# haiciyang/LaDiffCodec

Hardware: AMD Instinct MI355X
Metric: audio-sec decoded / wall-sec, 16kHz 3kbps 50-step DDPM (higher is better)
Workload: dtype bf16; 1 GPU; LaDiffCodec 3 kbps, diff_dims=256, enc_ratios 8 4, 50-step DDPM, batch=32x2.4 s utterances per GPU; global_batch=32, latent_len=1200, denoise_steps=50, rccl_ranks=1, batches_in_flight=1, parallelism=dp1 (utterance-sharded, no data-path collective)

## Files before the change

ladiffcodec_amd/csrc/attention.hip:

```cpp
#include <algorithm>

#include "ldc_kernels.h"
#include "ldc_math.h"

namespace ldc {

__device__ __forceinline__ float abf2f(unsigned short h) { return __uint_as_float(((unsigned)h) << 16); }
__device__ __forceinline__ unsigned short af2bf(float f) { return hw_bf16(f); }
template <typename T>
__device__ __forceinline__ float ld1(const void* p, size_t i);
template <>
__device__ __forceinline__ float ld1<float>(const void* p, size_t i) { return reinterpret_cast<const float*>(p)[i]; }
template <>
__device__ __forceinline__ float ld1<__bf16>(const void* p, size_t i) {
  return abf2f(reinterpret_cast<const unsigned short*>(p)[i]);
}
template <typename T>
__device__ __forceinline__ void st1(void* p, size_t i, float v);
template <>
__device__ __forceinline__ void st1<float>(void* p, size_t i, float v) { reinterpret_cast<float*>(p)[i] = v; }
template <>
__device__ __forceinline__ void st1<__bf16>(void* p, size_t i, float v) {
  reinterpret_cast<unsigned short*>(p)[i] = af2bf(v);
}
// ... 258 lines not shown
    }
    lf32x16 acc;
#pragma unroll
    for (int r = 0; r < 16; ++r) acc[r] = 0.f;
    acc = mfma_bf16(af[0], bq[0], acc);
    acc = mfma_bf16(af[1], bq[1], acc);
    if (n < L) {
      unsigned short* orow = out + ((size_t)b * L + n) * HD + h * D;
#pragma unroll
      for (int rr = 0; rr < 4; ++rr) {
        const unsigned lo = (unsigned)af2bf(acc[4 * rr]) | ((unsigned)af2bf(acc[4 * rr + 1]) << 16);
        const unsigned hi = (unsigned)af2bf(acc[4 * rr + 2]) | ((unsigned)af2bf(acc[4 * rr + 3]) << 16);
        *reinterpret_cast<uint2*>(orow + 8 * rr + 4 * g) = make_uint2(lo, hi);
      }
    }
  }
}


__device__ __forceinline__ float reduce16_over32(const float (&v)[16], int lane) {
  float a8[8], a4[4], a2[2];
  const bool b4 = lane & 16, b3 = lane & 8, b2 = lane & 4, b1 = lane & 2;
#pragma unroll
  for (int k = 0; k < 8; ++k) a8[k] = (b4 ? v[8 + k] : v[k]) + __shfl_xor(b4 ? v[k] : v[8 + k], 16);
#pragma unroll
  for (int k = 0; k < 4; ++k) a4[k] = (b3 ? a8[4 + k] : a8[k]) + __shfl_xor(b3 ? a8[k] : a8[4 + k], 8);
#pragma unroll
  for (int k = 0; k < 2; ++k) a2[k] = (b2 ? a4[2 + k] : a4[k]) + __shfl_xor(b2 ? a4[k] : a4[2 + k], 4);
  float a1 = (b1 ? a2[1] : a2[0]) + __shfl_xor(b1 ? a2[0] : a2[1], 2);
  a1 += __shfl_xor(a1, 1);
  return a1;
}

template <int C>
__global__ __launch_bounds__(256) void linattn_tail_mfma_kernel(const unsigned short* qkv, const float* ws, size_t ws_stride, float scale,
                                                                const unsigned short* wo, int n_pad, const float* bias, const float* gain,
                                                                const unsigned short* resid, unsigned short* out, int L) {
  constexpr int D = 32, HD = 128, R = 32, CPW = C / 4, NT = CPW / 32;
  constexpr int AP = HD + 8;
  constexpr int TP = CPW * 4 + 16;
  extern __shared__ __attribute__((aligned(16))) char smem[];
  unsigned short* sA = reinterpret_cast<unsigned short*>(smem);
  float* sred = reinterpret_cast<float*>(smem + (size_t)R * AP * 2);
  float* srow = sred + 4 * R;
  char* strans = smem + (size_t)R * AP * 2 + (size_t)5 * R * 4;
  const int b = blockIdx.y, tid = threadIdx.x;
  const int w = tid >> 6, lane = tid & 63, i32 = lane & 31, g = lane >> 5;
  const int r0 = blockIdx.x * R;
  const float* wsb = ws + (size_t)b * ws_stride;
  const int colw = w * CPW + i32;
  uint4 bfr[8][NT];
#pragma unroll
  for (int ks = 0; ks < 8; ++ks)
#pragma unroll
    for (int j = 0; j < NT; ++j)
      bfr[ks][j] = *reinterpret_cast<const uint4*>(wo + ((size_t)(ks >> 1) * n_pad + colw + 32 * j) * 32 + (ks & 1) * 16 + 8 * g);
  float bv[NT], gv[NT];
#pragma unroll
  for (int j = 0; j < NT; ++j) { bv[j] = bias[colw + 32 * j]; gv[j] = gain[colw + 32 * j]; }
  {
    const int h = w;
    const int n = r0 + i32;
    uint4 qq[2];
#pragma unroll
    for (int sx = 0; sx < 2; ++sx) {
      if (n < L) qq[sx] = *reinterpret_cast<const uint4*>(qkv + ((size_t)b * L + n) * (3 * HD) + h * D + 16 * sx + 8 * g);
      else qq[sx] = make_uint4(0, 0, 0, 0);
    }
    uint4 af[2];
#pragma unroll
    for (int sx = 0; sx < 2; ++sx) {
      unsigned wv[4];
#pragma unroll
      for (int m = 0; m < 8; m += 2) {
        const int d0 = 16 * sx + 8 * g + m;
        const float c0 = wsb[2 * HD + (size_t)h * D * D + d0 * D + i32] * (scale / wsb[HD + h * D + d0]);
        const float c1 = wsb[2 * HD + (size_t)h * D * D + (d0 + 1) * D + i32] * (scale / wsb[HD + h * D + d0 + 1]);
        wv[m >> 1] = (unsigned)af2bf(c0) | ((unsigned)af2bf(c1) << 16);
      }
      af[sx] = make_uint4(wv[0], wv[1], wv[2], wv[3]);
    }
    float x[16];
    float mx = -INFINITY;
#pragma unroll
    for (int sx = 0; sx < 2; ++sx) {
      const unsigned wv[4] = {qq[sx].x, qq[sx].y, qq[sx].z, qq[sx].w};
#pragma unroll
      for (int m = 0; m < 4; ++m) {
        x[8 * sx + 2 * m] = abf2f((unsigned short)(wv[m] & 0xffffu));
        x[8 * sx + 2 * m + 1] = abf2f((unsigned short)(wv[m] >> 16));
      }
    }
#pragma unroll
    for (int m = 0; m < 16; ++m) mx = fmaxf(mx, x[m]);
    mx = fmaxf(mx, __shfl_xor(mx, 32));
    float sum = 0.f;
#pragma unroll
    for (int m = 0; m < 16; ++m) { x[m] = __expf(x[m] - mx); sum += x[m]; }
    sum += __shfl_xor(sum, 32);
    const float inv = 1.0f / sum;
    uint4 bq[2];
#pragma unroll
    for (int sx = 0; sx < 2; ++sx) {
      unsigned wv[4];
#pragma unroll
      for (int m = 0; m < 4; ++m)
        wv[m] = (unsigned)af2bf(x[8 * sx + 2 * m] * inv) | ((unsigned)af2bf(x[8 * sx + 2 * m + 1] * inv) << 16);
      bq[sx] = make_uint4(wv[0], wv[1], wv[2], wv[3]);
    }
    lf32x16 acc1;
#pragma unroll
    for (int r = 0; r < 16; ++r) acc1[r] = 0.f;
    acc1 = mfma_bf16(af[0], bq[0], acc1);
    acc1 = mfma_bf16(af[1], bq[1], acc1);
    unsigned short* arow = sA + (size_t)i32 * AP + h * D;
#pragma unroll
    for (int rr = 0; rr < 4; ++rr) {
      const unsigned lo = (unsigned)af2bf(acc1[4 * rr]) | ((unsigned)af2bf(acc1[4 * rr + 1]) << 16);
      const unsigned hi = (unsigned)af2bf(acc1[4 * rr + 2]) | ((unsigned)af2bf(acc1[4 * rr + 3]) << 16);
      *reinterpret_cast<uint2*>(arow + 8 * rr + 4 * g) = make_uint2(lo, hi);
    }
  }
  __syncthreads();
  lf32x16 acc[NT];
#pragma unroll
  for (int j = 0; j < NT; ++j)
#pragma unroll
    for (int r = 0; r < 16; ++r) acc[j][r] = 0.f;
#pragma unroll
  for (int ks = 0; ks < 8; ++ks) {
    const uint4 afr = *reinterpret_cast<const uint4*>(sA + (size_t)i32 * AP + 16 * ks + 8 * g);
#pragma unroll
    for (int j = 0; j < NT; ++j) acc[j] = mfma_bf16(afr, bfr[ks][j], acc[j]);
  }
  constexpr int LPR = CPW / 4;
  constexpr int RPS = 64 / LPR;
  constexpr int NSW = R / RPS;
  const int rsub = lane / LPR, piece = lane % LPR;
  uint2 rres[NSW];
#pragma unroll
  for (int sw = 0; sw < NSW; ++sw) {
    const int n = r0 + sw * RPS + rsub;
    rres[sw] = n < L ? *reinterpret_cast<const uint2*>(resid + ((size_t)b * L + n) * C + w * CPW + piece * 4) : make_uint2(0, 0);
  }
#pragma unroll
  for (int j = 0; j < NT; ++j)
#pragma unroll
    for (int r = 0; r < 16; ++r) acc[j][r] += bv[j];
  const int rr = i32 >> 1;
  const int my_row = (rr & 3) + 8 * (rr >> 2) + 4 * g;
  {
    float v[16];
#pragma unroll
    for (int r = 0; r < 16; ++r) {
      float sacc = 0.f;
#pragma unroll
      for (int j = 0; j < NT; ++j) sacc += acc[j][r];
      v[r] = sacc;
    }
    const float tot = reduce16_over32(v, lane);
    if ((lane & 1) == 0) sred[w * R + my_row] = tot;
  }
  __syncthreads();
  if (tid < R) srow[tid] = (sred[tid] + sred[R + tid] + sred[2 * R + tid] + sred[3 * R + tid]) * (1.0f / (float)C);
  __syncthreads();
  float mean[16];
#pragma unroll
  for (int r = 0; r < 16; ++r) mean[r] = srow[(r & 3) + 8 * (r >> 2) + 4 * g];
  {
    float v[16];
#pragma unroll
    for (int r = 0; r < 16; ++r) {
      float sacc = 0.f;
#pragma unroll
      for (int j = 0; j < NT; ++j) { const float d = acc[j][r] - mean[r]; sacc = fmaf(d, d, sacc); }
      v[r] = sacc;
    }
    const float tot = reduce16_over32(v, lane);
    if ((lane & 1) == 0) sred[w * R + my_row] = tot;
  }
  __syncthreads();
  if (tid < R) srow[tid] = rsqrtf((sred[tid] + sred[R + tid] + sred[2 * R + tid] + sred[3 * R + tid]) * (1.0f / (float)C) + 1e-5f);
  __syncthreads();
  char* tw = strans + (size_t)w * R * TP;
#pragma unroll
  for (int r = 0; r < 16; ++r) {
    const int row = (r & 3) + 8 * (r >> 2) + 4 * g;
    const float rstd = srow[row];
#pragma unroll
    for (int j = 0; j < NT; ++j)
      reinterpret_cast<float*>(tw + (size_t)row * TP)[32 * j + i32] = (acc[j][r] - mean[r]) * rstd * gv[j];
  }
#pragma unroll
  for (int sw = 0; sw < NSW; ++sw) {
    const int row = sw * RPS + rsub;
    const int n = r0 + row;
    const float4 y = *reinterpret_cast<const float4*>(tw + (size_t)row * TP + piece * 16);
    const float o0 = y.x + abf2f((unsigned short)(rres[sw].x & 0xffffu)), o1 = y.y + abf2f((unsigned short)(rres[sw].x >> 16));
    const float o2 = y.z + abf2f((unsigned short)(rres[sw].y & 0xffffu)), o3 = y.w + abf2f((unsigned short)(rres[sw].y >> 16));
    const uint2 o = make_uint2((unsigned)af2bf(o0) | ((unsigned)af2bf(o1) << 16), (unsigned)af2bf(o2) | ((unsigned)af2bf(o3) << 16));
    if (n < L) *reinterpret_cast<uint2*>(out + ((size_t)b * L + n) * C + w * CPW + piece * 4) = o;
  }
}

template <int C>
static hipError_t launch_tail_cfg(const void* qkv, const float* ws, size_t wss, float scale, const void* wo, int n_pad, const float* bias,
                                  const float* gain, const void* resid, void* out, int B, int L, hipStream_t s) {
  constexpr int R = 32, CPW = C / 4;
  const size_t lds = (size_t)R * (128 + 8) * 2 + (size_t)5 * R * 4 + (size_t)4 * R * (CPW * 4 + 16);
  auto kern = linattn_tail_mfma_kernel<C>;
  static bool lds_opt_in = false;
  if (!lds_opt_in) {
    hipError_t e = hipFuncSetAttribute(reinterpret_cast<const void*>(kern), hipFuncAttributeMaxDynamicSharedMemorySize, 160 * 1024);
    if (e != hipSuccess) return e;
    lds_opt_in = true;
  }
  hipLaunchKernelGGL(kern, dim3((L + R - 1) / R, B), dim3(256), lds, s, reinterpret_cast<const unsigned short*>(qkv), ws, wss, scale,
                     reinterpret_cast<const unsigned short*>(wo), n_pad, bias, gain, reinterpret_cast<const unsigned short*>(resid),
                     reinterpret_cast<unsigned short*>(out), L);
  return hipGetLastError();
}

bool linattn_tail_supported(int dt, int heads, int dim_head, int C) {
  return dt == DT_BF16 && heads == 4 && dim_head == 32 && (C == 256 || C == 512 || C == 1024);
}

hipError_t launch_linattn_ctx(int dt, const void* qkv, float* ws, int B, int L, int heads, int dim_head, hipStream_t s) {
  if (dt != DT_BF16 || heads != 4 || dim_head != 32) return hipErrorInvalidValue;
  const size_t wss = linattn_ws_per_item(heads, dim_head);
  hipLaunchKernelGGL(linattn_ctx_mfma_kernel<64>, dim3((L + 63) / 64, B), dim3(256), 0, s, reinterpret_cast<const unsigned short*>(qkv), ws, L, wss);
  return hipGetLastError();
}

hipError_t launch_linattn_tail(int dt, const void* qkv, const float* ws, const void* wo_packed, int n_pad, const float* bias, const float* gain,
                               const void* resid, void* out, int B, int L, int heads, int dim_head, int C, hipStream_t s) {
  if (!linattn_tail_supported(dt, heads, dim_head, C) || !bias || !gain || !resid) return hipErrorInvalidValue;
  const size_t wss = linattn_ws_per_item(heads, dim_head);
  const float scale = 1.0f / sqrtf((float)dim_head);
  if (C == 256) return launch_tail_cfg<256>(qkv, ws, wss, scale, wo_packed, n_pad, bias, gain, resid, out, B, L, s);
  if (C == 512) return launch_tail_cfg<512>(qkv, ws, wss, scale, wo_packed, n_pad, bias, gain, resid, out, B, L, s);
  return launch_tail_cfg<1024>(qkv, ws, wss, scale, wo_packed, n_pad, bias, gain, resid, out, B, L, s);
}

size_t linattn_ws_floats_per_item(int heads, int dim_head) { return linattn_ws_per_item(heads, dim_head); }

hipError_t launch_linattn(int dt, const void* qkv, void* out, float* ws, int B, int L, int heads, int dim_head,
                          bool kmax_fused, hipStream_t s) {
  if (dim_head != 32 || heads * dim_head > 256 || 256 % (heads * dim_head) || 256 % heads) return hipErrorInvalidValue;
  const int HD = heads * dim_head;
  const size_t wss = linattn_ws_per_item(heads, dim_head);
  if (!kmax_fused) {
    hipError_t e = hipMemsetAsync(ws, 0, (size_t)B * wss * sizeof(float), s);
    if (e != hipSuccess) return e;
  }
  const int rpb = 128;
  const int chunks = (L + rpb - 1) / rpb;
  const float scale = 1.0f / sqrtf((float)dim_head);
  const size_t lds_out = (size_t)heads * (dim_head * dim_head + 8) * sizeof(float);
  const int rows_out = 256 / heads;
  if (dt == DT_BF16 && heads == 4) {
    if (!kmax_fused) hipLaunchKernelGGL(linattn_kmax_kernel<__bf16>, dim3(chunks, B), dim3(256), 0, s, qkv, ws, L, HD, rpb, wss);
    hipLaunchKernelGGL(linattn_ctx_mfma_kernel<64>, dim3((L + 63) / 64, B), dim3(256), 0, s,
                       reinterpret_cast<const unsigned short*>(qkv), ws, L, wss);
    hipLaunchKernelGGL(linattn_out_mfma_kernel<2>, dim3((L + 63) / 64, B), dim3(256), 0, s,
                       reinterpret_cast<const unsigned short*>(qkv), reinterpret_cast<unsigned short*>(out), ws, L, wss, scale);
  } else if (dt == DT_F32) {
    if (!kmax_fused) hipLaunchKernelGGL(linattn_kmax_kernel<float>, dim3(chunks, B), dim3(256), 0, s, qkv, ws, L, HD, rpb, wss);
    hipLaunchKernelGGL((linattn_ctx_kernel<float, 32>), dim3(chunks, B * heads), dim3(256), 0, s, qkv, ws, L, heads, rpb, wss);
    hipLaunchKernelGGL((linattn_out_kernel<float, 32>), dim3((L + rows_out - 1) / rows_out, B), dim3(256), lds_out, s, qkv,
                       out, ws, L, heads, wss, scale);
  } else {
// ... 101 lines not shown
```

ladiffcodec_amd/csrc/ldc_api.cpp:

```cpp
#include "ldc_internal.h"

long long g_device_syncs = 0;

static thread_local char g_err[1024] = "";
int fail(int code, const char* fmt, ...) {
  va_list ap;
  va_start(ap, fmt);
  vsnprintf(g_err, sizeof(g_err), fmt, ap);
  va_end(ap);
  return code;
}

extern "C" const char* ldc_last_error(void) { return g_err; }
extern "C" const char* ldc_version(void) { return "ladiffcodec-amd 0.1 (gfx950)"; }



static std::vector<float> fold_weight_norm(const HostTensor& g, const HostTensor& v) {
  const size_t n0 = (size_t)v.shape[0], inner = v.numel() / n0;
  std::vector<float> w(v.numel());
  for (size_t i = 0; i < n0; ++i) {
    double s = 0;
    for (size_t j = 0; j < inner; ++j) s += (double)v.data[i * inner + j] * v.data[i * inner + j];
    const float nrm = (float)sqrt(s);
// ... 747 lines not shown
}

extern "C" void ldc_quantize_e4m3(const float* in, int64_t n, uint8_t* out_codes, float* out_values) {
  for (int64_t i = 0; i < n; ++i) {
    const uint8_t q = host_f32_to_e4m3(in[i]);
    if (out_codes) out_codes[i] = q;
    if (out_values) out_values[i] = host_e4m3_to_f32(q);
  }
}

struct OptRef { int* p; bool replan; int lo, hi; };
static bool find_option(ldc_ctx* c, const std::string& n, OptRef* r) {
#define LDC_OPT(NAME, FIELD, REPLAN, LO, HI) if (n == NAME) { r->p = &(FIELD); r->replan = REPLAN; r->lo = LO; r->hi = HI; return true; }
  LDC_OPT("split", c->split_batch, true, 1, kMaxParts)
  LDC_OPT("part_graphs", c->part_graphs, false, 0, 2)
  LDC_OPT("graph_steps", c->graph_steps, false, 0, 1000)
  LDC_OPT("flow_depth", c->flow_depth, false, 0, (int)ldc_ctx::kFlowRing - 1)
  LDC_OPT("split_ends", c->split_ends, false, 0, 1)
  LDC_OPT("ends_join", c->ends_join, false, 0, 1)
  LDC_OPT("split_init", c->split_init, true, 0, 1)
  LDC_OPT("side_streams", c->side_streams, true, 0, 1)
  LDC_OPT("serial_parts", c->serial_parts, false, 0, 1)
  LDC_OPT("stream_calib", c->calib, false, 0, 1)
  LDC_OPT("merge_advance", c->merge_advance, true, 0, 1)
  LDC_OPT("fuse_gn_stats", c->fuse_gn_stats, true, 0, 1)
  LDC_OPT("fuse_gn_epi", c->fuse_gn_epi, true, 0, 1)
  LDC_OPT("gn_epi_min_l", c->gn_epi_min_l, true, 0, 1 << 30)
  LDC_OPT("gn_epi_max_tiles", c->gn_epi_max_tiles, true, 0, 1 << 30)
  LDC_OPT("fold_res", c->fold_res, true, 0, 1)
  LDC_OPT("fold_ln", c->fold_ln, true, 0, 1)
  LDC_OPT("fuse_kmax", c->fuse_kmax, true, 0, 1)
  LDC_OPT("fuse_ln", c->fuse_ln, true, 0, 1)
  LDC_OPT("fuse_attn_tail", c->fuse_attn_tail, true, 0, 1)
  LDC_OPT("fold_ctx", c->fold_ctx, true, 0, 1)
  LDC_OPT("conv_lean", c->tune.lean, true, 0, 1)
  LDC_OPT("conv_generic", c->tune.force_generic, true, 0, 1)
  LDC_OPT("conv_small_tiles", c->tune.small_max, true, 0, 1 << 30)
  LDC_OPT("conv_splitk", c->tune.splitk, true, 0, 4)
  LDC_OPT("sk_tiles", c->tune.sk_tiles, true, 0, 1 << 30)
  LDC_OPT("sk_u2", c->tune.sk_u2, true, 0, 1 << 30)
  LDC_OPT("sk_u3", c->tune.sk_u3, true, 0, 1 << 30)
  LDC_OPT("conv_mfast", c->tune.m_fastest, true, 0, 2)
  LDC_OPT("conv_debug", c->tune.debug, true, 0, 255)
  LDC_OPT("conv_tile", c->tune.force_tile, true, -1, 1)
  LDC_OPT("conv_xcd_order", c->tune.xcd_order, true, 0, 8)
  LDC_OPT("gn_nap", c->tune.gn_nap, true, 0, 4096)
  LDC_OPT("gn_nap0", c->tune.gn_nap0, true, 0, 4096)
  LDC_OPT("lstm_stream", c->lstm_stream_only, false, 0, 1)
  LDC_OPT("lstm_xcd", c->lstm_xcd, false, 0, 1)
  LDC_OPT("lstm_pipe", c->lstm_pipe, false, 0, 1)
  LDC_OPT("coop_launch", c->coop_launch, false, 0, 1)
  LDC_OPT("sea_splitk", c->sea_splitk, false, 0, 1)
  LDC_OPT("rvq_tiled", c->rvq_tiled, false, 0, 1)
  LDC_OPT("train_bf16", g_train_bf16, false, 0, 1)
  LDC_OPT("train_fp32_mfma", g_train_fp32_mfma, false, 0, 1)
  LDC_OPT("train_valu", g_train_valu, false, 0, 1)
  LDC_OPT("train_dw_side", g_train_dw_side, false, 0, 1)
#undef LDC_OPT
  return false;
}

extern "C" int ldc_set_option(ldc_ctx* c, const char* name, int value) {
  if (!c || !name) return fail(LDC_E_INVALID, "null context or option name");
  const std::string n(name);
  if (n == "fp8_act") {
    if (c->finalized) return fail(LDC_E_STATE, "fp8_act must be set before ldc_finalize_weights");
// ... 642 lines not shown
    int t[4];
    conv_bm(a.qkv_ln, L, L, false, t);
    return t[0] > 0;
  }
  void* attention(const LinAttnW& a, const void* x, int L, bool linear, void* xn_pre = nullptr) {
    const int rows = B * L, dt = c->dt, Bn = B;
    const int H = c->unet.heads, Dh = c->unet.dim_head, hid = H * Dh;
    const bool f8 = qkv_fp8(a);
    const bool lnf = !xn_pre && ln_foldable(a, L);
    const float* rowstat = lnf ? last_rowstat : nullptr;
    last_rowstat = nullptr;
    void* xn = lnf ? const_cast<void*>(x) : (xn_pre ? xn_pre : (f8 ? ar->alloc((size_t)rows * a.dim) : act(rows, a.dim)));
    const ConvLayer& qkv_ly = lnf ? a.qkv_ln : (f8 ? a.qkv_f8 : a.qkv);
    void* qkv = act(rows, 3 * hid);
    void* o = act(rows, hid);
    void* out = act(rows, a.dim);
    const LinAttnW* ap = &a;
    float* ws = (linear && c->fuse_kmax) ? linattn_ws + (size_t)(linattn_used++) * B * linattn_ws_floats_per_item(H, Dh) : linattn_ws;
    if (!xn_pre && !lnf)
      add([=](hipStream_t s) { return launch_ln_rows(dt, x, xn, nullptr, ap->norm_g, rows, ap->dim, s, f8 ? 1 : 0); }, false, 0, LDC_CLASS_LAYERNORM,
          2.0 * rows * a.dim * es);
    if (linear) {
      const size_t wss = linattn_ws_floats_per_item(H, Dh);
      if (c->fuse_kmax && c->fuse_attn_tail && !a.out.w8 && linattn_tail_supported(dt, H, Dh, a.dim)) {
        ln_rowstat_next = rowstat;
        if (lnf && c->fold_ctx && c->tune.lean && !c->tune.force_generic && dt == DT_BF16 && a.qkv_ctx.w && hid == 128 && a.dim % 64 == 0) {
          qkv_ctx_next = ws; qkv_ctx_stride_next = (int)wss;
          conv(a.qkv_ctx, xn, nullptr, qkv, nullptr, L, L);
        } else {
          conv(qkv_ly, xn, nullptr, qkv, nullptr, L, L, nullptr, reinterpret_cast<unsigned*>(ws), hid, 2 * hid, (int)wss);
          add([=](hipStream_t s) { return launch_linattn_ctx(dt, qkv, ws, Bn, L, H, Dh, s); }, false, 0, LDC_CLASS_LINATTN, 2.0 * rows * hid * es);
        }
        const int dim = a.dim;
        info = "tail_c" + std::to_string(dim) + "_L" + std::to_string(L) + "_B" + std::to_string(B);
        add([=](hipStream_t s) {
          return launch_linattn_tail(dt, qkv, ws, ap->out.w, ap->out.n_pad, ap->out.bias, ap->out_g, x, out, Bn, L, H, Dh, dim, s);
        }, false, 2.0 * rows * hid * dim, LDC_CLASS_LINATTN, (1.0 * hid + 2.0 * dim) * rows * es);
        return out;
      }
      if (c->fuse_kmax) {
        ln_rowstat_next = rowstat;
        conv(qkv_ly, xn, nullptr, qkv, nullptr, L, L, nullptr, reinterpret_cast<unsigned*>(ws), hid, 2 * hid, (int)wss);
        add([=](hipStream_t s) { return launch_linattn(dt, qkv, o, ws, Bn, L, H, Dh, true, s); }, false, 0, LDC_CLASS_LINATTN,
            4.0 * rows * hid * es);
      } else {
        ln_rowstat_next = rowstat;
        conv(qkv_ly, xn, nullptr, qkv, nullptr, L, L);
        add([=](hipStream_t s) { return launch_linattn(dt, qkv, o, ws, Bn, L, H, Dh, false, s); }, false, 0, LDC_CLASS_LINATTN,
            5.0 * rows * hid * es);
      }
      void* t = act(rows, a.dim);
      conv(a.out, o, nullptr, t, nullptr, L, L);
      add([=](hipStream_t s) { return launch_ln_rows(dt, t, out, x, ap->out_g, rows, ap->dim, s); }, false, 0, LDC_CLASS_LAYERNORM,
          3.0 * rows * a.dim * es);
    } else {
      ln_rowstat_next = rowstat;
      conv(qkv_ly, xn, nullptr, qkv, nullptr, L, L);
      add([=](hipStream_t s) { return launch_attn_full(dt, qkv, o, Bn, L, H, Dh, s); }, false, 0, LDC_CLASS_ATTN_FULL, 4.0 * rows * hid * es);
      conv(a.out, o, nullptr, out, x, L, L);
    }
    return out;
  }
};

int build_plan(ldc_ctx* c, Plan* pl, Arena& ar, int B, int L, int F) {
  const UnetW& u = c->unet;
  pl->B = B; pl->L = L; pl->F = F;
  pl->cond_ops.clear(); pl->step_ops.clear(); pl->step_is_conv.clear(); pl->step_where.clear(); pl->step_flops.clear(); pl->step_class.clear(); pl->step_bytes.clear(); pl->step_info.clear(); pl->taps.clear();
  pl->flops = 0; pl->act_bytes = 0; pl->conv_bytes = 0; pl->sk_need_max = 0; pl->part_need = 0;
// ... 1019 lines not shown
```

ladiffcodec_amd/csrc/ldc_internal.h:

```cpp
#pragma once
#include "../../include/ladiffcodec.h"

#include <hip/hip_runtime.h>
#include <math.h>
#include <stdarg.h>
#include <stdio.h>
#include <string.h>

#include <algorithm>
#include <chrono>
#include <functional>
#include <map>
#include <memory>
#include <set>
#include <string>
#include <vector>

#include "ldc_kernels.h"

extern long long g_device_syncs;
inline hipError_t counted_device_sync() {
  ++g_device_syncs;
  return hipDeviceSynchronize();
}
// ... 219 lines not shown
  Halves last_halves;
  hipStream_t aux_stream[kMaxParts] = {nullptr, nullptr, nullptr, nullptr};
  hipEvent_t ev_fork = nullptr, ev_join[kMaxParts] = {nullptr, nullptr, nullptr, nullptr};
  static constexpr int kLstmChunks = 4;
  hipEvent_t lstm_ev[kMaxParts][kLstmChunks + 1] = {};
  hipStream_t calib_stream = nullptr; bool calibrated = false;
  int calib_good = -1, calib_cand = 0; double calib_one_ms = 0, calib_all_ms = 0;
  struct CalibOrder { hipStream_t s; std::vector<hipStream_t> order; int good, cand; double one_ms, all_ms; };
  std::vector<CalibOrder> calib_cache;
  int calib = 1;
  int ends_join = 0;
  int lstm_pipe = 0;
  int split_batch = 2;
  int merge_advance = 1;
  int rvq_tiled = 1;
  int sea_splitk = 1;
  int split_init = 1;
  int split_ends = 1;
  int fp8_act = 1;
  int part_graphs = 1;
  double host_graph_ms = 0, host_wait_ms = 0;
  long long host_graph_launches = 0;
  hipStream_t side_stream[kMaxParts] = {nullptr, nullptr, nullptr, nullptr};
  hipEvent_t ev_side_fork[kMaxParts] = {nullptr, nullptr, nullptr, nullptr}, ev_side_join[kMaxParts] = {nullptr, nullptr, nullptr, nullptr};
  int side_streams = 0;
  int fuse_kmax = 1;
  int fuse_ln = 1;
  int coop_launch = 0;
  int lstm_xcd = 1;
  int num_cus = 256;
  int xcd_resident[2] = {0, 0};
  int coop_resident[2] = {0, 0};
  int fuse_attn_tail = 1;
  int fold_ctx = 1;
  static constexpr int kFlowRing = 32;
  hipEvent_t flow_ev[kFlowRing] = {};
  unsigned long long flow_n = 0;
  int flow_depth = 8;
  int fuse_gn_stats = 1;
  int gn_epi_max_tiles = 1300;
  int gn_epi_min_l = 0;
  int fold_ln = 1;
  int fold_res = 1;
  int fuse_gn_epi = 1;
  ConvTune tune;
  int lstm_stream_only = 0;
  int serial_parts = 0;
  int graph_steps = 0;
  uint64_t use_tick = 0, call_tick = 0;
  size_t plan_bytes = 0, plan_bytes_cap = (size_t)48 << 30;
  int plan_count_cap = 24;
  uint64_t noise_epoch = 0, cur_key = 0;
  unsigned* dev_flag_host = nullptr;
  unsigned* dev_flag_dev = nullptr;
  int enc_final_act = ACT_NONE;
  unsigned long long* tl_buf = nullptr;
  bool timeline = false;
  bool kstamps = false;
  char* scratch = nullptr;
  size_t scratch_cap = 0;
  void* outnorm_ws = nullptr;
  size_t outnorm_ws_bytes = 0;
  float* state_buf = nullptr;
  size_t state_bytes = 0;
  hipStream_t own_stream = nullptr;
  bool profile = false;
// ... 110 lines not shown
```

ladiffcodec_amd/csrc/ldc_kernels.h:

```cpp
#pragma once
#include <hip/hip_runtime.h>
#include <stdint.h>

namespace ldc {

enum { DT_F32 = 0, DT_BF16 = 1, DT_FP8 = 2 };
enum { ACT_NONE = 0, ACT_SILU = 1, ACT_ELU = 2, ACT_TANH = 3, ACT_GELU = 4, ACT_SIGMOID = 5, ACT_RELU = 6 };
enum { PAD_ZERO = 0, PAD_REFLECT = 1 };
static constexpr int kGnPad = 16;

inline size_t dt_size(int dt) { return dt == DT_F32 ? 4 : (dt == DT_FP8 ? 1 : 2); }

struct ConvLayer {
  int dt = DT_F32;
  int cin1 = 0, cin2 = 0;
  int n = 0;
  int n_pad = 0;
  int bn = 128;
  int taps = 1, stride = 1, dil = 1, pad_left = 0, ups = 0, pad_mode = PAD_ZERO;
  int pre_act = ACT_NONE, post_act = ACT_NONE;
  int tr_stride = 0, tr_cout = 0, tr_trim_left = 0;
  void* w = nullptr;
  float* bias = nullptr;
  int w8 = 0;
// ... 52 lines not shown
  const int* kst_step = nullptr;
  int kst_stride = 0;
  const ConvTune* tune = nullptr;
  long long* sk_need = nullptr;
  int* bm_out = nullptr;
};

hipError_t launch_conv(const ConvLayer& ly, const ConvCall& c, hipStream_t s);
long long conv_generic_splitk_floats(const ConvLayer& ly, const ConvCall& c);
size_t conv_packed_weight_bytes(const ConvLayer& ly);
void pack_conv_weights(const ConvLayer& ly, const float* w_oik, void* dst_host);
void pack_conv_weights_fp8(const ConvLayer& ly, const float* w_oik, void* dst_host, float* scales);
void pack_conv_weights_fp8act(const ConvLayer& ly, const float* w_oik, void* dst_host, float* scales);
uint8_t host_f32_to_e4m3(float f);
float host_e4m3_to_f32(uint8_t v);
void pack_convtr_weights(const ConvLayer& ly, const float* w_iok, int cin, int cout, int stride, void* dst_host);
int conv_pick_bn(int n);

hipError_t launch_gn_stats(int dt, const void* x, int B, int L, int C, int groups, float* stats, hipStream_t s);
hipError_t launch_gn_apply(int dt, const void* x, void* y, const void* residual, int B, int L, int C, int groups,
                           const float* stats, const float* gamma, const float* beta, const float* ss_table,
                           int ss_stride, const int* t_ptr, int act, hipStream_t s, void* y_ln = nullptr, const float* ln_g = nullptr, int out8 = 0);
bool gn_apply_ln_fusable(int C);
hipError_t launch_ln_rows(int dt, const void* x, void* y, const void* residual, const float* g, int rows, int C,
                          hipStream_t s, int out8 = 0);
hipError_t launch_act(int dt, const void* x, void* y, int64_t n, int act, hipStream_t s, int out8 = 0);

hipError_t launch_linattn(int dt, const void* qkv, void* out, float* ctx_ws, int B, int L, int heads, int dim_head,
                          bool kmax_fused, hipStream_t s);
size_t linattn_ws_floats_per_item(int heads, int dim_head);
bool linattn_tail_supported(int dt, int heads, int dim_head, int C);
hipError_t launch_linattn_ctx(int dt, const void* qkv, float* ctx_ws, int B, int L, int heads, int dim_head, hipStream_t s);
hipError_t launch_linattn_tail(int dt, const void* qkv, const float* ctx_ws, const void* wo_packed, int n_pad, const float* bias, const float* gain,
                               const void* resid, void* out, int B, int L, int heads, int dim_head, int C, hipStream_t s);
hipError_t launch_attn_full(int dt, const void* qkv, void* out, int B, int L, int heads, int dim_head, hipStream_t s);

hipError_t launch_to_cl(int dt, const float* x_bcl, void* y_blc, int B, int C, int L, const float* maxabs,
                        int maxabs_per_item, float eps, hipStream_t s);
hipError_t launch_from_cl(int dt, const void* x_blc, float* y_bcl, int B, int C, int L, const float* maxabs,
                          int maxabs_per_item, float eps, hipStream_t s);
hipError_t launch_maxabs(int dt, const void* x, int B, int64_t n_per_item, int per_item, float* maxabs,
                         hipStream_t s);
struct StepTables {
  const float* sqrt_recip_alphas_cumprod;
  const float* sqrt_recipm1_alphas_cumprod;
  const float* posterior_mean_coef1;
  const float* posterior_mean_coef2;
  const float* posterior_log_variance_clipped;
};
hipError_t launch_random_fill(float* x, int64_t n, int uniform, uint64_t seed, unsigned step, hipStream_t s);
hipError_t launch_axpby(float* x, const float* y, float a, float b, int64_t n, hipStream_t s);
hipError_t launch_p_sample_update(int dt, float* x, const void* eps_cl, const float* noise, int64_t noise_step_stride,
                                  void* x_cl, int B, int C, int L, StepTables tb, const int* st,
                                  uint64_t elem_base, hipStream_t s);
struct DdimStep {
  int t;
  int last;
  float sqrt_an;
  float c;
  float sigma;
  float pad_[3];
};
hipError_t launch_ddim_table_write(DdimStep* dst, const DdimStep* src_host, int n, hipStream_t s);
hipError_t launch_ddim_update(int dt, float* x, const void* eps_cl, const float* noise, int64_t noise_step_stride,
                              void* x_cl, int B, int C, int L, StepTables tb, const DdimStep* sched, const int* st,
                              uint64_t elem_base, hipStream_t s);
hipError_t launch_scale_by_maxabs(int dt, void* x, int B, int64_t n_per_item, const float* maxabs, int per_item,
// ... 106 lines not shown
```

Baseline: 614.3 audio-s/wall-s.

## Stream linear-attention tail output weights through an LDS ring via async global-to-LDS loads

Adds a variant of the fused linear-attention tail kernel that no longer preloads the whole output-projection weight slice into registers. Each wave now streams 32-column weight slices into a per-wave multi-stage LDS ring using global_load_lds_dwordx4, with vmcnt waits, so the next slice's load overlaps MFMAs on the current one. The aim is lower register pressure and more hidden weight-load latency. The cost is more LDS use (raised opt-in limit), fragile inline asm that touches m0, and XOR-swizzled LDS addressing that has to match exactly. The shared head and layernorm code is factored into helpers, and the new path is on by default through an option.

```diff
diff --git a/ladiffcodec_amd/csrc/attention.hip b/ladiffcodec_amd/csrc/attention.hip
--- a/ladiffcodec_amd/csrc/attention.hip
+++ b/ladiffcodec_amd/csrc/attention.hip
@@ -314,13 +314,155 @@
   return a1;
 }
 
+template <int AP>
+__device__ __forceinline__ void tail_heads_to_lds(const unsigned short* qkv, const float* wsb, float scale, unsigned short* sA, int b,
+                                                  int r0, int L, int h, int i32, int g) {
+  constexpr int D = 32, HD = 128;
+  const int n = r0 + i32;
+  uint4 qq[2];
+#pragma unroll
+  for (int sx = 0; sx < 2; ++sx) {
+    if (n < L) qq[sx] = *reinterpret_cast<const uint4*>(qkv + ((size_t)b * L + n) * (3 * HD) + h * D + 16 * sx + 8 * g);
+    else qq[sx] = make_uint4(0, 0, 0, 0);
+  }
+  uint4 af[2];
+#pragma unroll
+  for (int sx = 0; sx < 2; ++sx) {
+    unsigned wv[4];
+#pragma unroll
+    for (int m = 0; m < 8; m += 2) {
+      const int d0 = 16 * sx + 8 * g + m;
+      const float c0 = wsb[2 * HD + (size_t)h * D * D + d0 * D + i32] * (scale / wsb[HD + h * D + d0]);
+      const float c1 = wsb[2 * HD + (size_t)h * D * D + (d0 + 1) * D + i32] * (scale / wsb[HD + h * D + d0 + 1]);
+      wv[m >> 1] = (unsigned)af2bf(c0) | ((unsigned)af2bf(c1) << 16);
+    }
+    af[sx] = make_uint4(wv[0], wv[1], wv[2], wv[3]);
+  }
+  float x[16];
+  float mx = -INFINITY;
+#pragma unroll
+  for (int sx = 0; sx < 2; ++sx) {
+    const unsigned wv[4] = {qq[sx].x, qq[sx].y, qq[sx].z, qq[sx].w};
+#pragma unroll
+    for (int m = 0; m < 4; ++m) {
+      x[8 * sx + 2 * m] = abf2f((unsigned short)(wv[m] & 0xffffu));
+      x[8 * sx + 2 * m + 1] = abf2f((unsigned short)(wv[m] >> 16));
+    }
+  }
+#pragma unroll
+  for (int m = 0; m < 16; ++m) mx = fmaxf(mx, x[m]);
+  mx = fmaxf(mx, __shfl_xor(mx, 32));
+  float sum = 0.f;
+#pragma unroll
+  for (int m = 0; m < 16; ++m) { x[m] = __expf(x[m] - mx); sum += x[m]; }
+  sum += __shfl_xor(sum, 32);
+  const float inv = 1.0f / sum;
+  uint4 bq[2];
+#pragma unroll
+  for (int sx = 0; sx < 2; ++sx) {
+    unsigned wv[4];
+#pragma unroll
+    for (int m = 0; m < 4; ++m)
+      wv[m] = (unsigned)af2bf(x[8 * sx + 2 * m] * inv) | ((unsigned)af2bf(x[8 * sx + 2 * m + 1] * inv) << 16);
+    bq[sx] = make_uint4(wv[0], wv[1], wv[2], wv[3]);
+  }
+  lf32x16 acc1;
+#pragma unroll
+  for (int r = 0; r < 16; ++r) acc1[r] = 0.f;
+  acc1 = mfma_bf16(af[0], bq[0], acc1);
+  acc1 = mfma_bf16(af[1], bq[1], acc1);
+  unsigned short* arow = sA + (size_t)i32 * AP + h * D;
+#pragma unroll
+  for (int rr = 0; rr < 4; ++rr) {
+    const unsigned lo = (unsigned)af2bf(acc1[4 * rr]) | ((unsigned)af2bf(acc1[4 * rr + 1]) << 16);
+    const unsigned hi = (unsigned)af2bf(acc1[4 * rr + 2]) | ((unsigned)af2bf(acc1[4 * rr + 3]) << 16);
+    *reinterpret_cast<uint2*>(arow + 8 * rr + 4 * g) = make_uint2(lo, hi);
+  }
+}
+
+template <int C>
+__device__ __forceinline__ void tail_ln_store(lf32x16 (&acc)[C / 128], const float (&bv)[C / 128], const float (&gv)[C / 128], float* sred,
+                                              float* srow, char* strans, const unsigned short* resid, unsigned short* out, int b, int r0,
+                                              int L, int w, int lane, int tid) {
+  constexpr int R = 32, CPW = C / 4, NT = CPW / 32;
+  constexpr int TP = CPW * 4 + 16;
+  const int i32 = lane & 31, g = lane >> 5;
+  constexpr int LPR = CPW / 4;
+  constexpr int RPS = 64 / LPR;
+  constexpr int NSW = R / RPS;
+  const int rsub = lane / LPR, piece = lane % LPR;
+  uint2 rres[NSW];
+#pragma unroll
+  for (int sw = 0; sw < NSW; ++sw) {
+    const int n = r0 + sw * RPS + rsub;
+    rres[sw] = n < L ? *reinterpret_cast<const uint2*>(resid + ((size_t)b * L + n) * C + w * CPW + piece * 4) : make_uint2(0, 0);
+  }
+#pragma unroll
+  for (int j = 0; j < NT; ++j)
+#pragma unroll
+    for (int r = 0; r < 16; ++r) acc[j][r] += bv[j];
+  const int rr = i32 >> 1;
+  const int my_row = (rr & 3) + 8 * (rr >> 2) + 4 * g;
+  {
+    float v[16];
+#pragma unroll
+    for (int r = 0; r < 16; ++r) {
+      float sacc = 0.f;
+#pragma unroll
+      for (int j = 0; j < NT; ++j) sacc += acc[j][r];
+      v[r] = sacc;
+    }
+    const float tot = reduce16_over32(v, lane);
+    if ((lane & 1) == 0) sred[w * R + my_row] = tot;
+  }
+  __syncthreads();
+  if (tid < R) srow[tid] = (sred[tid] + sred[R + tid] + sred[2 * R + tid] + sred[3 * R + tid]) * (1.0f / (float)C);
+  __syncthreads();
+  float mean[16];
+#pragma unroll
+  for (int r = 0; r < 16; ++r) mean[r] = srow[(r & 3) + 8 * (r >> 2) + 4 * g];
+  {
+    float v[16];
+#pragma unroll
+    for (int r = 0; r < 16; ++r) {
+      float sacc = 0.f;
+#pragma unroll
+      for (int j = 0; j < NT; ++j) { const float d = acc[j][r] - mean[r]; sacc = fmaf(d, d, sacc); }
+      v[r] = sacc;
+    }
+    const float tot = reduce16_over32(v, lane);
+    if ((lane & 1) == 0) sred[w * R + my_row] = tot;
+  }
+  __syncthreads();
+  if (tid < R) srow[tid] = rsqrtf((sred[tid] + sred[R + tid] + sred[2 * R + tid] + sred[3 * R + tid]) * (1.0f / (float)C) + 1e-5f);
+  __syncthreads();
+  char* tw = strans + (size_t)w * R * TP;
+#pragma unroll
+  for (int r = 0; r < 16; ++r) {
+    const int row = (r & 3) + 8 * (r >> 2) + 4 * g;
+    const float rstd = srow[row];
+#pragma unroll
+    for (int j = 0; j < NT; ++j)
+      reinterpret_cast<float*>(tw + (size_t)row * TP)[32 * j + i32] = (acc[j][r] - mean[r]) * rstd * gv[j];
+  }
+#pragma unroll
+  for (int sw = 0; sw < NSW; ++sw) {
+    const int row = sw * RPS + rsub;
+    const int n = r0 + row;
+    const float4 y = *reinterpret_cast<const float4*>(tw + (size_t)row * TP + piece * 16);
+    const float o0 = y.x + abf2f((unsigned short)(rres[sw].x & 0xffffu)), o1 = y.y + abf2f((unsigned short)(rres[sw].x >> 16));
+    const float o2 = y.z + abf2f((unsigned short)(rres[sw].y & 0xffffu)), o3 = y.w + abf2f((unsigned short)(rres[sw].y >> 16));
+    const uint2 o = make_uint2((unsigned)af2bf(o0) | ((unsigned)af2bf(o1) << 16), (unsigned)af2bf(o2) | ((unsigned)af2bf(o3) << 16));
+    if (n < L) *reinterpret_cast<uint2*>(out + ((size_t)b * L + n) * C + w * CPW + piece * 4) = o;
+  }
+}
+
 template <int C>
 __global__ __launch_bounds__(256) void linattn_tail_mfma_kernel(const unsigned short* qkv, const float* ws, size_t ws_stride, float scale,
                                                                 const unsigned short* wo, int n_pad, const float* bias, const float* gain,
                                                                 const unsigned short* resid, unsigned short* out, int L) {
-  constexpr int D = 32, HD = 128, R = 32, CPW = C / 4, NT = CPW / 32;
+  constexpr int HD = 128, R = 32, CPW = C / 4, NT = CPW / 32;
   constexpr int AP = HD + 8;
-  constexpr int TP = CPW * 4 + 16;
   extern __shared__ __attribute__((aligned(16))) char smem[];
   unsigned short* sA = reinterpret_cast<unsigned short*>(smem);
   float* sred = reinterpret_cast<float*>(smem + (size_t)R * AP * 2);
@@ -340,69 +482,7 @@
   float bv[NT], gv[NT];
 #pragma unroll
   for (int j = 0; j < NT; ++j) { bv[j] = bias[colw + 32 * j]; gv[j] = gain[colw + 32 * j]; }
-  {
-    const int h = w;
-    const int n = r0 + i32;
-    uint4 qq[2];
-#pragma unroll
-    for (int sx = 0; sx < 2; ++sx) {
-      if (n < L) qq[sx] = *reinterpret_cast<const uint4*>(qkv + ((size_t)b * L + n) * (3 * HD) + h * D + 16 * sx + 8 * g);
-      else qq[sx] = make_uint4(0, 0, 0, 0);
-    }
-    uint4 af[2];
-#pragma unroll
-    for (int sx = 0; sx < 2; ++sx) {
-      unsigned wv[4];
-#pragma unroll
-      for (int m = 0; m < 8; m += 2) {
-        const int d0 = 16 * sx + 8 * g + m;
-        const float c0 = wsb[2 * HD + (size_t)h * D * D + d0 * D + i32] * (scale / wsb[HD + h * D + d0]);
-        const float c1 = wsb[2 * HD + (size_t)h * D * D + (d0 + 1) * D + i32] * (scale / wsb[HD + h * D + d0 + 1]);
-        wv[m >> 1] = (unsigned)af2bf(c0) | ((unsigned)af2bf(c1) << 16);
-      }
-      af[sx] = make_uint4(wv[0], wv[1], wv[2], wv[3]);
-    }
-    float x[16];
-    float mx = -INFINITY;
-#pragma unroll
-    for (int sx = 0; sx < 2; ++sx) {
-      const unsigned wv[4] = {qq[sx].x, qq[sx].y, qq[sx].z, qq[sx].w};
-#pragma unroll
-      for (int m = 0; m < 4; ++m) {
-        x[8 * sx + 2 * m] = abf2f((unsigned short)(wv[m] & 0xffffu));
-        x[8 * sx + 2 * m + 1] = abf2f((unsigned short)(wv[m] >> 16));
-      }
-    }
-#pragma unroll
-    for (int m = 0; m < 16; ++m) mx = fmaxf(mx, x[m]);
-    mx = fmaxf(mx, __shfl_xor(mx, 32));
-    float sum = 0.f;
-#pragma unroll
-    for (int m = 0; m < 16; ++m) { x[m] = __expf(x[m] - mx); sum += x[m]; }
-    sum += __shfl_xor(sum, 32);
-    const float inv = 1.0f / sum;
-    uint4 bq[2];
-#pragma unroll
-    for (int sx = 0; sx < 2; ++sx) {
-      unsigned wv[4];
-#pragma unroll
-      for (int m = 0; m < 4; ++m)
-        wv[m] = (unsigned)af2bf(x[8 * sx + 2 * m] * inv) | ((unsigned)af2bf(x[8 * sx + 2 * m + 1] * inv) << 16);
-      bq[sx] = make_uint4(wv[0], wv[1], wv[2], wv[3]);
-    }
-    lf32x16 acc1;
-#pragma unroll
-    for (int r = 0; r < 16; ++r) acc1[r] = 0.f;
-    acc1 = mfma_bf16(af[0], bq[0], acc1);
-    acc1 = mfma_bf16(af[1], bq[1], acc1);
-    unsigned short* arow = sA + (size_t)i32 * AP + h * D;
-#pragma unroll
-    for (int rr = 0; rr < 4; ++rr) {
-      const unsigned lo = (unsigned)af2bf(acc1[4 * rr]) | ((unsigned)af2bf(acc1[4 * rr + 1]) << 16);
-      const unsigned hi = (unsigned)af2bf(acc1[4 * rr + 2]) | ((unsigned)af2bf(acc1[4 * rr + 3]) << 16);
-      *reinterpret_cast<uint2*>(arow + 8 * rr + 4 * g) = make_uint2(lo, hi);
-    }
-  }
+  tail_heads_to_lds<AP>(qkv, wsb, scale, sA, b, r0, L, w, i32, g);
   __syncthreads();
   lf32x16 acc[NT];
 #pragma unroll
@@ -415,74 +495,98 @@
 #pragma unroll
     for (int j = 0; j < NT; ++j) acc[j] = mfma_bf16(afr, bfr[ks][j], acc[j]);
   }
-  constexpr int LPR = CPW / 4;
-  constexpr int RPS = 64 / LPR;
-  constexpr int NSW = R / RPS;
-  const int rsub = lane / LPR, piece = lane % LPR;
-  uint2 rres[NSW];
-#pragma unroll
-  for (int sw = 0; sw < NSW; ++sw) {
-    const int n = r0 + sw * RPS + rsub;
-    rres[sw] = n < L ? *reinterpret_cast<const uint2*>(resid + ((size_t)b * L + n) * C + w * CPW + piece * 4) : make_uint2(0, 0);
-  }
+  tail_ln_store<C>(acc, bv, gv, sred, srow, strans, resid, out, b, r0, L, w, lane, tid);
+}
+
+template <int N>
+__device__ __forceinline__ void tail_wait_vmcnt() {
+  static_assert(N >= 0 && N <= 63, "vmcnt is six bits");
+  asm volatile("s_waitcnt vmcnt(%0)" ::"n"(N) : "memory");
+}
+
+__device__ __forceinline__ void tail_slice_dma(const unsigned short* wo, int n_pad, int ch0, int lane, unsigned stage) {
+  const int i = lane >> 2, s = lane & 3;
+  const unsigned voff = (unsigned)((i * 32 + (s ^ ((i >> 2) & 3)) * 8) * 2);
+#pragma unroll
+  for (int ck = 0; ck < 4; ++ck) {
+#pragma unroll
+    for (int half = 0; half < 2; ++half) {
+      const char* base = reinterpret_cast<const char*>(wo + ((size_t)ck * n_pad + ch0 + 16 * half) * 32);
+      const unsigned m0v = stage + (unsigned)(ck * 2048 + half * 1024);
+      unsigned keep;
+      asm volatile("s_mov_b32 %0, m0\n\ts_mov_b32 m0, %3\n\ts_nop 0\n\tglobal_load_lds_dwordx4 %1, %2\n\ts_mov_b32 m0, %0"
+                   : "=&s"(keep)
+                   : "v"(voff), "s"(base), "s"(m0v)
+                   : "memory");
+    }
+  }
+}
+
+template <int NT, int S, int J>
+__device__ __forceinline__ void tail_wait_slice() {
+  constexpr int last = J - 1 + S < NT - 1 ? J - 1 + S : NT - 1;
+  tail_wait_vmcnt<8 * (last - J)>();
+}
+
+template <int C, int NT, int S, int J>
+__device__ __forceinline__ void tail_stream_steps(lf32x16 (&acc)[NT], const uint4 (&afr)[8], const unsigned short* wo, int n_pad, int w,
+                                                  int i32, int g, int lane, unsigned ring, const char* ring_ptr) {
+  if constexpr (J < NT) {
+    constexpr int CPW = C / 4;
+    tail_wait_slice<NT, S, J>();
+    const char* st = ring_ptr + (J % S) * 8192;
+#pragma unroll
+    for (int ks = 0; ks < 8; ++ks) {
+      const int slot = ((ks & 1) * 2 + g) ^ ((i32 >> 2) & 3);
+      const uint4 bf = *reinterpret_cast<const uint4*>(st + (ks >> 1) * 2048 + i32 * 64 + slot * 16);
+      acc[J] = mfma_bf16(afr[ks], bf, acc[J]);
+    }
+    if constexpr (J + S < NT) {
+      asm volatile("s_waitcnt lgkmcnt(0)" ::: "memory");
+      tail_slice_dma(wo, n_pad, w * CPW + 32 * (J + S), lane, ring + (unsigned)((J % S) * 8192));
+    }
+    tail_stream_steps<C, NT, S, J + 1>(acc, afr, wo, n_pad, w, i32, g, lane, ring, ring_ptr);
+  }
+}
+
+template <int C, int S>
+__global__ __launch_bounds__(256) void linattn_tail_stream_kernel(const unsigned short* qkv, const float* ws, size_t ws_stride, float scale,
+                                                                  const unsigned short* wo, int n_pad, const float* bias, const float* gain,
+                                                                  const unsigned short* resid, unsigned short* out, int L) {
+  typedef __attribute__((address_space(3))) void* lptr_t;
+  constexpr int HD = 128, R = 32, CPW = C / 4, NT = CPW / 32;
+  constexpr int AP = HD + 8;
+  constexpr int RING = 4 * S * 8192, TRANS = 4 * R * (CPW * 4 + 16);
+  constexpr int BIG = RING > TRANS ? RING : TRANS;
+  static_assert(S >= 1 && S <= NT, "ring stages");
+  extern __shared__ __attribute__((aligned(16))) char smem[];
+  char* sring = smem;
+  unsigned short* sA = reinterpret_cast<unsigned short*>(smem + BIG);
+  float* sred = reinterpret_cast<float*>(smem + BIG + (size_t)R * AP * 2);
+  float* srow = sred + 4 * R;
+  const int b = blockIdx.y, tid = threadIdx.x;
+  const int w = __builtin_amdgcn_readfirstlane(tid >> 6), lane = tid & 63, i32 = lane & 31, g = lane >> 5;
+  const int r0 = blockIdx.x * R;
+  const float* wsb = ws + (size_t)b * ws_stride;
+  const int colw = w * CPW + i32;
+  float bv[NT], gv[NT];
+#pragma unroll
+  for (int j = 0; j < NT; ++j) { bv[j] = bias[colw + 32 * j]; gv[j] = gain[colw + 32 * j]; }
+  const unsigned ring = (unsigned)(size_t)(lptr_t)sring + (unsigned)(w * S * 8192);
+  tail_heads_to_lds<AP>(qkv, wsb, scale, sA, b, r0, L, w, i32, g);
+#pragma unroll
+  for (int j = 0; j < S; ++j) tail_slice_dma(wo, n_pad, w * CPW + 32 * j, lane, ring + (unsigned)(j * 8192));
+  __syncthreads();
+  uint4 afr[8];
+#pragma unroll
+  for (int ks = 0; ks < 8; ++ks) afr[ks] = *reinterpret_cast<const uint4*>(sA + (size_t)i32 * AP + 16 * ks + 8 * g);
+  lf32x16 acc[NT];
 #pragma unroll
   for (int j = 0; j < NT; ++j)
 #pragma unroll
-    for (int r = 0; r < 16; ++r) acc[j][r] += bv[j];
-  const int rr = i32 >> 1;
-  const int my_row = (rr & 3) + 8 * (rr >> 2) + 4 * g;
-  {
-    float v[16];
-#pragma unroll
-    for (int r = 0; r < 16; ++r) {
-      float sacc = 0.f;
-#pragma unroll
-      for (int j = 0; j < NT; ++j) sacc += acc[j][r];
-      v[r] = sacc;
-    }
-    const float tot = reduce16_over32(v, lane);
-    if ((lane & 1) == 0) sred[w * R + my_row] = tot;
-  }
-  __syncthreads();
-  if (tid < R) srow[tid] = (sred[tid] + sred[R + tid] + sred[2 * R + tid] + sred[3 * R + tid]) * (1.0f / (float)C);
-  __syncthreads();
-  float mean[16];
-#pragma unroll
-  for (int r = 0; r < 16; ++r) mean[r] = srow[(r & 3) + 8 * (r >> 2) + 4 * g];
-  {
-    float v[16];
-#pragma unroll
-    for (int r = 0; r < 16; ++r) {
-      float sacc = 0.f;
-#pragma unroll
-      for (int j = 0; j < NT; ++j) { const float d = acc[j][r] - mean[r]; sacc = fmaf(d, d, sacc); }
-      v[r] = sacc;
-    }
-    const float tot = reduce16_over32(v, lane);
-    if ((lane & 1) == 0) sred[w * R + my_row] = tot;
-  }
-  __syncthreads();
-  if (tid < R) srow[tid] = rsqrtf((sred[tid] + sred[R + tid] + sred[2 * R + tid] + sred[3 * R + tid]) * (1.0f / (float)C) + 1e-5f);
-  __syncthreads();
-  char* tw = strans + (size_t)w * R * TP;
-#pragma unroll
-  for (int r = 0; r < 16; ++r) {
-    const int row = (r & 3) + 8 * (r >> 2) + 4 * g;
-    const float rstd = srow[row];
-#pragma unroll
-    for (int j = 0; j < NT; ++j)
-      reinterpret_cast<float*>(tw + (size_t)row * TP)[32 * j + i32] = (acc[j][r] - mean[r]) * rstd * gv[j];
-  }
-#pragma unroll
-  for (int sw = 0; sw < NSW; ++sw) {
-    const int row = sw * RPS + rsub;
-    const int n = r0 + row;
-    const float4 y = *reinterpret_cast<const float4*>(tw + (size_t)row * TP + piece * 16);
-    const float o0 = y.x + abf2f((unsigned short)(rres[sw].x & 0xffffu)), o1 = y.y + abf2f((unsigned short)(rres[sw].x >> 16));
-    const float o2 = y.z + abf2f((unsigned short)(rres[sw].y & 0xffffu)), o3 = y.w + abf2f((unsigned short)(rres[sw].y >> 16));
-    const uint2 o = make_uint2((unsigned)af2bf(o0) | ((unsigned)af2bf(o1) << 16), (unsigned)af2bf(o2) | ((unsigned)af2bf(o3) << 16));
-    if (n < L) *reinterpret_cast<uint2*>(out + ((size_t)b * L + n) * C + w * CPW + piece * 4) = o;
-  }
+    for (int r = 0; r < 16; ++r) acc[j][r] = 0.f;
+  tail_stream_steps<C, NT, S, 0>(acc, afr, wo, n_pad, w, i32, g, lane, ring, sring + (size_t)w * S * 8192);
+  tail_ln_store<C>(acc, bv, gv, sred, srow, sring, resid, out, b, r0, L, w, lane, tid);
 }
 
 template <int C>
@@ -503,6 +607,25 @@
   return hipGetLastError();
 }
 
+template <int C>
+static hipError_t launch_tail_stream_cfg(const void* qkv, const float* ws, size_t wss, float scale, const void* wo, int n_pad,
+                                         const float* bias, const float* gain, const void* resid, void* out, int B, int L, hipStream_t s) {
+  constexpr int R = 32, CPW = C / 4, S = C == 1024 ? 4 : C == 512 ? 2 : 1;
+  constexpr size_t RING = (size_t)4 * S * 8192, TRANS = (size_t)4 * R * (CPW * 4 + 16);
+  const size_t lds = std::max(RING, TRANS) + (size_t)R * (128 + 8) * 2 + (size_t)5 * R * 4;
+  auto kern = linattn_tail_stream_kernel<C, S>;
+  static bool lds_opt_in = false;
+  if (!lds_opt_in) {
+    hipError_t e = hipFuncSetAttribute(reinterpret_cast<const void*>(kern), hipFuncAttributeMaxDynamicSharedMemorySize, 160 * 1024);
+    if (e != hipSuccess) return e;
+    lds_opt_in = true;
+  }
+  hipLaunchKernelGGL(kern, dim3((L + R - 1) / R, B), dim3(256), lds, s, reinterpret_cast<const unsigned short*>(qkv), ws, wss, scale,
+                     reinterpret_cast<const unsigned short*>(wo), n_pad, bias, gain, reinterpret_cast<const unsigned short*>(resid),
+                     reinterpret_cast<unsigned short*>(out), L);
+  return hipGetLastError();
+}
+
 bool linattn_tail_supported(int dt, int heads, int dim_head, int C) {
   return dt == DT_BF16 && heads == 4 && dim_head == 32 && (C == 256 || C == 512 || C == 1024);
 }
@@ -515,10 +638,15 @@
 }
 
 hipError_t launch_linattn_tail(int dt, const void* qkv, const float* ws, const void* wo_packed, int n_pad, const float* bias, const float* gain,
-                               const void* resid, void* out, int B, int L, int heads, int dim_head, int C, hipStream_t s) {
+                               const void* resid, void* out, int B, int L, int heads, int dim_head, int C, bool stream, hipStream_t s) {
   if (!linattn_tail_supported(dt, heads, dim_head, C) || !bias || !gain || !resid) return hipErrorInvalidValue;
   const size_t wss = linattn_ws_per_item(heads, dim_head);
   const float scale = 1.0f / sqrtf((float)dim_head);
+  if (stream) {
+    if (C == 256) return launch_tail_stream_cfg<256>(qkv, ws, wss, scale, wo_packed, n_pad, bias, gain, resid, out, B, L, s);
+    if (C == 512) return launch_tail_stream_cfg<512>(qkv, ws, wss, scale, wo_packed, n_pad, bias, gain, resid, out, B, L, s);
+    return launch_tail_stream_cfg<1024>(qkv, ws, wss, scale, wo_packed, n_pad, bias, gain, resid, out, B, L, s);
+  }
   if (C == 256) return launch_tail_cfg<256>(qkv, ws, wss, scale, wo_packed, n_pad, bias, gain, resid, out, B, L, s);
   if (C == 512) return launch_tail_cfg<512>(qkv, ws, wss, scale, wo_packed, n_pad, bias, gain, resid, out, B, L, s);
   return launch_tail_cfg<1024>(qkv, ws, wss, scale, wo_packed, n_pad, bias, gain, resid, out, B, L, s);
diff --git a/ladiffcodec_amd/csrc/ldc_api.cpp b/ladiffcodec_amd/csrc/ldc_api.cpp
--- a/ladiffcodec_amd/csrc/ldc_api.cpp
+++ b/ladiffcodec_amd/csrc/ldc_api.cpp
@@ -803,6 +803,7 @@
   LDC_OPT("fuse_kmax", c->fuse_kmax, true, 0, 1)
   LDC_OPT("fuse_ln", c->fuse_ln, true, 0, 1)
   LDC_OPT("fuse_attn_tail", c->fuse_attn_tail, true, 0, 1)
+  LDC_OPT("attn_tail_stream", c->attn_tail_stream, true, 0, 1)
   LDC_OPT("fold_ctx", c->fold_ctx, true, 0, 1)
   LDC_OPT("conv_lean", c->tune.lean, true, 0, 1)
   LDC_OPT("conv_generic", c->tune.force_generic, true, 0, 1)
@@ -1511,9 +1512,10 @@
           add([=](hipStream_t s) { return launch_linattn_ctx(dt, qkv, ws, Bn, L, H, Dh, s); }, false, 0, LDC_CLASS_LINATTN, 2.0 * rows * hid * es);
         }
         const int dim = a.dim;
+        const bool stream = c->attn_tail_stream != 0;
         info = "tail_c" + std::to_string(dim) + "_L" + std::to_string(L) + "_B" + std::to_string(B);
         add([=](hipStream_t s) {
-          return launch_linattn_tail(dt, qkv, ws, ap->out.w, ap->out.n_pad, ap->out.bias, ap->out_g, x, out, Bn, L, H, Dh, dim, s);
+          return launch_linattn_tail(dt, qkv, ws, ap->out.w, ap->out.n_pad, ap->out.bias, ap->out_g, x, out, Bn, L, H, Dh, dim, stream, s);
         }, false, 2.0 * rows * hid * dim, LDC_CLASS_LINATTN, (1.0 * hid + 2.0 * dim) * rows * es);
         return out;
       }
diff --git a/ladiffcodec_amd/csrc/ldc_internal.h b/ladiffcodec_amd/csrc/ldc_internal.h
--- a/ladiffcodec_amd/csrc/ldc_internal.h
+++ b/ladiffcodec_amd/csrc/ldc_internal.h
@@ -275,6 +275,7 @@
   int xcd_resident[2] = {0, 0};
   int coop_resident[2] = {0, 0};
   int fuse_attn_tail = 1;
+  int attn_tail_stream = 1;
   int fold_ctx = 1;
   static constexpr int kFlowRing = 32;
   hipEvent_t flow_ev[kFlowRing] = {};
diff --git a/ladiffcodec_amd/csrc/ldc_kernels.h b/ladiffcodec_amd/csrc/ldc_kernels.h
--- a/ladiffcodec_amd/csrc/ldc_kernels.h
+++ b/ladiffcodec_amd/csrc/ldc_kernels.h
@@ -108,7 +108,7 @@
 bool linattn_tail_supported(int dt, int heads, int dim_head, int C);
 hipError_t launch_linattn_ctx(int dt, const void* qkv, float* ctx_ws, int B, int L, int heads, int dim_head, hipStream_t s);
 hipError_t launch_linattn_tail(int dt, const void* qkv, const float* ctx_ws, const void* wo_packed, int n_pad, const float* bias, const float* gain,
-                               const void* resid, void* out, int B, int L, int heads, int dim_head, int C, hipStream_t s);
+                               const void* resid, void* out, int B, int L, int heads, int dim_head, int C, bool stream, hipStream_t s);
 hipError_t launch_attn_full(int dt, const void* qkv, void* out, int B, int L, int heads, int dim_head, hipStream_t s);
 
 hipError_t launch_to_cl(int dt, const float* x_bcl, void* y_blc, int B, int C, int L, const float* maxabs,
```

Result: no change. 613.9 audio-s/wall-s (median of 2 runs) (-0.1%).
